# whh1747012859/Enhanced-UNet

Measured on AMD Instinct MI355X. Metric: training images/sec at 1024×1024 1-ch→2-cls, 1/2/4/8 MI355X; Dice vs CPU ref, higher is better.
Workload: dtype bf16

## Files before the change

### enhanced-unet_amd/csrc/bn_pool_up.hip

```cpp
#include "common.h"

#include <algorithm>

EUNET_DEBUG_UNIT(bnpool)

namespace {

constexpr int NT = 256;
constexpr int STH = 8, STW = 32;
constexpr int SFH = 16;
constexpr int SCI = 8;
constexpr int SJT = (SCI * 9 + 15) / 16;

struct SmallArgs {
  const void* x; int N, H, W, xct, xco, cin;
  const float* w; const float* b;
  void* y; int yct, yco, cout;
  float* stats; int tx, ty, ntiles;
};

template <typename T, bool C1>
__global__ __launch_bounds__(NT) void conv_small_fwd_kernel(SmallArgs a) {
  __shared__ float xs[(SFH + 2) * (STW + 2) * SCI];
  __shared__ __attribute__((aligned(16))) float wsm[SCI * 9 * 64];
// ... 341 lines not shown
  if (tid == 0 && c == 0 && nbt != nullptr) *nbt += 1;
  if (tid == 0) {
    const double var_b = m2 / n;
    const double var_u = n > 1.0 ? m2 / (n - 1.0) : var_b;
    const double istd = 1.0 / sqrt(var_b + (double)eps);
    const double sc = (double)gamma[c] * istd;
    if (mean_o) mean_o[c] = (float)mean;
    if (invstd_o) invstd_o[c] = (float)istd;
    if (scale_o) scale_o[c] = (float)sc;
    if (shift_o) shift_o[c] = (float)((double)beta[c] - mean * sc);
    if (rm) rm[c] = (float)((1.0 - mom) * (double)rm[c] + mom * mean);
    if (rv) rv[c] = (float)((1.0 - mom) * (double)rv[c] + mom * var_u);
  }
}

__global__ void bn_eval_affine_kernel(int C, const float* g, const float* b, const float* rm, const float* rv,
                                      float eps, float* sc, float* sh) {
  const int c = blockIdx.x * blockDim.x + threadIdx.x;
  if (c >= C) return;
  const float s = g[c] / sqrtf(rv[c] + eps);
  sc[c] = s;
  sh[c] = b[c] - rm[c] * s;
}

template <typename T>
__global__ void bnrelu_pool_kernel(const T* y, int N, int H, int W, int C, int yct, int yco, const float* sc,
                                   const float* sh, T* act, int act_ct, int act_co, T* pool, int pct, int pco) {
  constexpr int E = Vec16<T>::N;
  const int U = C / E, Ho = H / 2, Wo = W / 2;
  const long long id = (long long)blockIdx.x * blockDim.x + threadIdx.x;
// ... 306 lines not shown
  const int col = blockIdx.x * 64 + cl;
  double s = 0.0;
  if (col < cols) {
    for (int r = rg; r < rb; r += 32) {
      double v[8];
#pragma unroll
      for (int i = 0; i < 8; ++i) {
        const double x = ws[(long long)min(r + 4 * i, rb - 1) * cols + col];
        v[i] = r + 4 * i < rb ? x : 0.0;
      }
#pragma unroll
      for (int i = 0; i < 8; ++i) s += v[i];
    }
  }
  sh[rg][cl] = s;
  __syncthreads();
  if (rg == 0 && col < cols) {
    const float v = (float)(sh[0][cl] + sh[1][cl] + sh[2][cl] + sh[3][cl]);
    int i = 0;
#pragma unroll
    for (int j = 1; j < 4; ++j) i = (j < segs.n && col >= segs.start[j]) ? j : i;
    segs.out[i][col - segs.start[i]] = v;
  }
}

struct BnBwdCoef { float k1, kq, k2, k3; };
__device__ __forceinline__ BnBwdCoef bn_bwd_coef(float mean, float istd, float scale, float shift, float dbeta,
                                                 float dgamma, float inv_n) {
  const float off = -mean * istd;
  const float dg = dgamma * inv_n;
// ... 628 lines not shown
  for (int i = 0; i < segs.n; ++i)
    EUNET_REQUIRE(segs.out[i] && (i == 0 || (segs.start[i] > segs.start[i - 1] && segs.start[i] < cols)),
                  "colsum: bad segments");
  const int rb = colsum_rb(rows);
  const int chunk = cdiv(rows, rb);
  colsum_stage1<<<dim3(cdiv(cols, 64), rb), NT, 0, s>>>(part, rows, cols, ld, chunk, (double*)ws);
  colsum_stage2<<<cdiv(cols, 64), NT, 0, s>>>((const double*)ws, rb, cols, segs);
  EUNET_LAUNCH_CHECK("colsum");
  return EUNET_OK;
}

int eunet_colsum_ld(const float* part, int rows, int cols, int ld, float* out, void* ws, hipStream_t s, int split,
                    float* out_hi) {
  ColSegs g = {{out, out_hi, nullptr, nullptr}, {0, split, 0, 0}, out_hi != nullptr ? 2 : 1};
  return eunet_colsum_segs(part, rows, cols, ld, g, ws, s);
}

namespace {
int bnr_block(const eunet_act* g) {
  const int U = g->c / elems16(g->dtype);
  return U > 0 && NT % U == 0 ? NT : (U > 0 && 192 % U == 0 ? 192 : 0);
}
bool bnr_ok(const eunet_act* g, const eunet_act* y) {
  return act_ok(y) && vec_ok(y) && like(y, g) && bnr_block(g) > 0;
}
long long pool_threads(const eunet_act* gout) {
  return (long long)gout->n * (gout->h / 2) * (gout->w / 2) * (gout->c / elems16(gout->dtype));
}
int bnr_grid(long long threads, int cap, int block) { return (int)std::min<long long>((threads + block - 1) / block, cap); }
long long up_threads(const eunet_act* glo) {
// ... 212 lines not shown
  });
  EUNET_LAUNCH_CHECK("bn_bwd_reduce");
  return EUNET_OK;
}

int eunet_colsum_ws_bytes(int rows, int cols, size_t* bytes) {
  EUNET_REQUIRE(bytes && rows > 0 && cols > 0, "colsum_ws_bytes: bad args");
  *bytes = eunet_colsum_ws(rows, cols);
  return EUNET_OK;
}

int eunet_colsum(const float* part, int rows, int cols, float* out, void* ws, void* stream) {
  return eunet_colsum_ld(part, rows, cols, cols, out, ws, (hipStream_t)stream);
}

int eunet_colsum_split(const float* part, int rows, int cols, int split, float* out_lo, float* out_hi, void* ws,
                       void* stream) {
  EUNET_REQUIRE(out_hi && split > 0 && split < cols, "colsum_split: bad split");
  return eunet_colsum_ld(part, rows, cols, cols, out_lo, ws, (hipStream_t)stream, split, out_hi);
}

int eunet_bn_bwd_apply(const eunet_act* g, const eunet_act* y, const float* mean, const float* invstd,
                       const float* scale, const float* shift, const float* dbeta, const float* dgamma,
                       const eunet_act* gy, void* stream) {
  EUNET_REQUIRE(act_ok(g) && act_ok(y) && act_ok(gy) && vec_ok(g) && vec_ok(y) && vec_ok(gy),
                "bn_bwd_apply: bad tensors");
  EUNET_REQUIRE(mean && invstd && scale && shift && dbeta && dgamma, "bn_bwd_apply: null stats");
  EUNET_REQUIRE(like(g, y) && like(gy, y), "bn_bwd_apply: mismatch");
  const long long P = (long long)y->n * y->h * y->w;
  const int U = y->c / elems16(y->dtype);
// ... 171 lines not shown
```

### enhanced-unet_amd/csrc/common.h

```cpp
#pragma once
#include <hip/hip_runtime.h>

#include <mutex>
#include <utility>
#include <vector>
#include <stdint.h>
#include <stdio.h>
#include <string.h>

#include "../../include/eunet.h"

typedef __bf16 bf16x8 __attribute__((ext_vector_type(8)));
typedef short s16x4 __attribute__((ext_vector_type(4)));
typedef short s16x8 __attribute__((ext_vector_type(8)));
typedef float f32x4 __attribute__((ext_vector_type(4)));
typedef uint32_t u32x4 __attribute__((ext_vector_type(4)));
typedef float f32x2 __attribute__((ext_vector_type(2)));
typedef short s16x2 __attribute__((ext_vector_type(2)));
typedef uint16_t bf16_t;

__device__ __forceinline__ bf16x8 cat_bf16x4(s16x4 lo, s16x4 hi) {
  const s16x8 v = __builtin_shufflevector(lo, hi, 0, 1, 2, 3, 4, 5, 6, 7);
  return __builtin_bit_cast(bf16x8, v);
}
// ... 167 lines not shown
  f32x4 w = {0.25f, 0.75f, 0.75f, 0.25f};
  if (i == 0) { w[0] = 0.f; w[1] = 1.f; }
  if (i == in - 1) { w[2] = 1.f; w[3] = 0.f; }
  return w;
}

int eunet_colsum_ld(const float* part, int rows, int cols, int ld, float* out, void* ws, hipStream_t s,
                    int split = 0, float* out_hi = nullptr);
struct ColSegs {
  float* out[4];
  int start[4];
  int n;
};
int eunet_colsum_segs(const float* part, int rows, int cols, int ld, const ColSegs& segs, void* ws, hipStream_t s);

template <typename K>
inline void allow_lds(K* kernel, size_t bytes) {
  if (bytes <= 65536) return;
  static std::mutex mu;
  static std::vector<std::pair<const void*, size_t>> done;
  std::lock_guard<std::mutex> lock(mu);
  for (const auto& d : done)
    if (d.first == (const void*)kernel && d.second >= bytes) return;
  (void)hipFuncSetAttribute((const void*)kernel, hipFuncAttributeMaxDynamicSharedMemorySize, (int)bytes);
  done.emplace_back((const void*)kernel, bytes);
}

__host__ __device__ inline int cdiv(int a, int b) { return (a + b - 1) / b; }

inline bool act_ok(const eunet_act* a) {
// ... 27 lines not shown
```

### enhanced-unet_amd/eunet/_lib.py

```python
from __future__ import annotations

import ctypes
import os
from ctypes import POINTER, c_float, c_int, c_size_t, c_void_p, c_char_p, c_int64

LIB_PATH = os.environ.get("EUNET_LIB") or os.path.join(os.path.dirname(os.path.abspath(__file__)), "libeunet_hip.so")

EUNET_F32 = 0
EUNET_BF16 = 1


class Act(ctypes.Structure):
    _fields_ = [("ptr", c_void_p), ("n", c_int), ("h", c_int), ("w", c_int), ("c", c_int),
                ("ctot", c_int), ("coff", c_int), ("dtype", c_int)]


class PackDesc(ctypes.Structure):
    _fields_ = [("w", c_void_p), ("cout", c_int), ("cin", c_int), ("flip", c_int), ("wp", c_void_p)]


PACK_MAX = 32


class LossParams(ctypes.Structure):
# ... 82 lines not shown
    "eunet_bce_dice_bwd": [_f, _f, c_int, c_int, c_int, c_int, POINTER(BCEDiceParams), _f, _f, _f, c_void_p],
    "eunet_border_weight_map": [_f, _f, c_int, c_int, c_int, POINTER(c_float * 3), c_float, c_float, c_int, _f, c_void_p],
    "eunet_separate_instances": [_f, _f, c_int, c_int, c_int, _f, _f, c_void_p],
    "eunet_loss_fwd_w": [_f, _f, _f, c_int, c_int, c_int, c_int, POINTER(LossParams), _f, _f, _f, _f, c_void_p],
    "eunet_loss_bwd_w": [_f, _f, _f, c_int, c_int, c_int, c_int, POINTER(LossParams), _f, _f, _f, c_void_p],
    "eunet_bce_dice_fwd_w": [_f, _f, _f, c_int, c_int, c_int, c_int, POINTER(BCEDiceParams), _f, _f, _f, _f, c_void_p],
    "eunet_bce_dice_bwd_w": [_f, _f, _f, c_int, c_int, c_int, c_int, POINTER(BCEDiceParams), _f, _f, _f, c_void_p],
    "eunet_warp_grid": [_f, c_int, c_int, POINTER(ctypes.c_double * 6), c_int, c_int, _f, c_void_p],
    "eunet_warp_u8": [_f, c_int, c_int, c_int, _f, c_int, c_int, c_int, c_int, _f, c_void_p],
    "eunet_warp_labels": [_f, c_int, c_int, c_int, c_int, _f, c_int, c_int, c_int, c_int64, c_int, c_int, _f, c_void_p],
    "eunet_bn_bwd_tiles": [_P, POINTER(c_int)],
    "eunet_bn_bwd_reduce": [_P, _P, _f, _f, _f, _f, _f, c_void_p],
    "eunet_colsum_ws_bytes": [c_int, c_int, POINTER(c_size_t)],
    "eunet_colsum": [_f, c_int, c_int, _f, _f, c_void_p],
    "eunet_colsum_split": [_f, c_int, c_int, c_int, _f, _f, _f, c_void_p],
    "eunet_bn_bwd_apply": [_P, _P, _f, _f, _f, _f, _f, _f, _P, c_void_p],
    "eunet_bn_bwd_apply_1x1": [_P, _f, c_int, _f, _f, _f, _f, _f, _f, _f, _P, c_void_p],
    "eunet_pool_bwd_add": [_P, _P, _P, _P, c_void_p],
    "eunet_upsample_bwd": [_P, _P, c_void_p],
    "eunet_pool_bwd_add_bnr_rows": [_P, POINTER(c_int)],
    "eunet_pool_bwd_add_bnr": [_P, _P, _P, _P, _P, _f, _f, _f, _f, _f, c_void_p],
    "eunet_bn_bwd_apply_pool": [_P, _P, _P, _f, _f, _f, _f, _f, _f, _P, c_void_p],
    "eunet_upsample_bwd_bnr_rows": [_P, POINTER(c_int)],
    "eunet_upsample_bwd_bnr": [_P, _P, _P, _f, _f, _f, _f, _f, c_void_p],
    "eunet_conv1x1_bwd_tiles": [_P, POINTER(c_int)],
    "eunet_conv1x1_bwd": [_P, _f, _f, _f, c_int, _f, _P, _f, c_void_p],
    "eunet_conv1x1_bwd_bnr": [_P, _f, _f, _f, c_int, _f, _P, _f, _f, _f, _f, c_void_p],
    "eunet_semantic_counts": [_f, _f, c_int, c_int64, _f, c_void_p],
    "eunet_binary_overlap": [_f, _f, c_int64, _f, c_void_p],
    "eunet_resize_bilinear": [_f, c_int, c_int, c_int, _f, c_int, c_int, c_float, c_float, c_int, c_int,
# ... 166 lines not shown
```

### enhanced-unet_amd/eunet/dual.py

```python
from __future__ import annotations

from typing import List, Optional

import torch

from . import ops
from .engine import BN_EPS, BN_MOMENTUM, GradSink, UNetEngine, _e

DROP_P = (0.2, 0.15)
HEAD_CH = (256, 128, 64)
BRANCHES = ("unetpp", "deeplab")


class DualEngine:
    narrow_mfma = True

    def __init__(self, model):
        self.m = model
        self.K = model.num_classes
        self.ea = UNetEngine(model, prefix="unetpp.")
        self.eb = UNetEngine(model, prefix="deeplab.")
        self.drop_keep = None
        self.keep_state = False

# ... 73 lines not shown
        else:
            keep = torch.empty((N, C), dtype=torch.float32, device=dev).bernoulli_(1.0 - DROP_P[i])
        sc, sh, gs = (_e((N, C), torch.float32, dev) for _ in range(3))
        ops.dropout_affine(h["scale"], h["shift"], keep, DROP_P[i], sc, sh, gs)
        return dict(scale=sc, shift=sh, nstride=C, gscale=gs)

    def _bn_back(self, prefix, g, y, bn, P, sink, part=None, tiles=0):
        C = y.shape[3]
        dev = y.device
        if part is None:
            tiles = ops.bn_bwd_tiles(ops.act(y))
            part = _e(tiles * 2 * C, torch.float32, dev)
            ops.bn_bwd_reduce(ops.act(g), ops.act(y), bn["mean"], bn["invstd"], bn["scale"],
                              bn["shift"], part)
        dbeta, dgamma = sink.slot(prefix + ".bias", (C,)), sink.slot(prefix + ".weight", (C,))
        ops.colsum(part, tiles, 2 * C, dbeta, split=C, out_hi=dgamma)
        gy = torch.empty_like(y)
        ops.bn_bwd_apply(ops.act(g), ops.act(y), bn["mean"], bn["invstd"], bn["scale"],
                         bn["shift"], dbeta, dgamma, ops.act(gy))
        return gy

    def _wgrad(self, name, xa: ops.Act, gy, sink, d=None):
        C = gy.shape[3]
        dev = gy.device
        gya = ops.act(gy)
        ns = ops.conv3x3_wgrad_splits(gya, xa.c, self.dtype)
        dwp = _e(ns * C * 9 * xa.c, torch.float32, dev)
        ops.conv3x3_wgrad(xa, gya, dwp, None, ns, scale=d["scale"], shift=d["shift"], nstride=d["nstride"])
        ops.wgrad_reduce(dwp, None, ns, C, xa.c, 9, sink.slot(name, (C, xa.c, 3, 3)), None)

    def backward(self, S, g_out, g_aux_a, g_aux_b, sink: Optional[GradSink] = None):
# ... 2 lines not shown
        N, H, W = S["N"], S["H"], S["W"]
        dev = g_out.device
        sink = sink or GradSink(dev)
        za, zb = S["SA"]["z"], S["SB"]["z"]
        tiles, gtiles = ops.fusion_tiles(N, H, W)
        g1, g2, h1, h2, h3, d1, d2 = (S[k] for k in ("g1", "g2", "h1", "h2", "h3", "d1", "d2"))
        y1, y2, y3, a, b, f2 = (S[k] for k in ("y1", "y2", "y3", "a", "b", "f2"))
        g_out = g_out.contiguous().float()
        gz = _e((N, H, W, K), torch.float32, dev)
        gf2res = _e((N, H, W, 2 * K), torch.float32, dev)
        nv = K * 2 * K + K
        part = _e(tiles * nv, torch.float32, dev)
        ops.fusion_out_bwd(za, zb, K, g_out, b, g2["scale"], g2["shift"],
                           P["fusion_residual.weight"].reshape(K, 2 * K).contiguous(), gz, gf2res, part)
        red = _e(nv, torch.float32, dev)
        ops.colsum(part, tiles, nv, red)
        sink.slot("fusion_residual.weight", (K, 2 * K, 1, 1)).copy_(red[:2 * K * K].view(K, 2 * K, 1, 1))
        sink.slot("fusion_residual.bias", (K,)).copy_(red[2 * K * K:])
        C3 = HEAD_CH[2]
        g3 = torch.empty_like(y3)
        ct = ops.conv1x1_bwd_tiles(ops.act(y3))
        part = _e(ct * (K * C3 + K), torch.float32, dev)
        w11 = P["fusion_head.11.weight"].reshape(K, C3).contiguous()
        bpart = _e(ct * 2 * C3, torch.float32, dev)
        ops.conv1x1_bwd_bnr(ops.act(y3), h3["scale"], h3["shift"], w11, K, gz, ops.act(g3), part,
                            h3["mean"], h3["invstd"], bpart)
        red = _e(K * C3 + K, torch.float32, dev)
        ops.colsum(part, ct, K * C3 + K, red)
        sink.slot("fusion_head.11.weight", (K, C3, 1, 1)).copy_(red[:K * C3].view(K, C3, 1, 1))
        sink.slot("fusion_head.11.bias", (K,)).copy_(red[K * C3:])
        sink.ready(["fusion_residual.weight", "fusion_residual.bias", "fusion_head.11.weight", "fusion_head.11.bias"])
        gy3 = self._bn_back("fusion_head.9", g3, y3, h3, P, sink, part=bpart, tiles=ct)
        del g3
        self._wgrad("fusion_head.8.weight", ops.act(y2), gy3, sink, d2)
        gg2 = torch.empty_like(y2)
        ct = ops.conv3x3_tiles(ops.act(gg2))
        cpart = _e(ct * 2 * HEAD_CH[1], torch.float32, dev)
        ops.conv3x3_dgrad_bnbwd(ops.act(gy3), ops.conv3x3_pack(P["fusion_head.8.weight"], dt, flip=True),
                                ops.act(gg2), ops.act(y2), h2["mean"], h2["invstd"], h2["scale"],
                                h2["shift"], cpart, gscale=d2["gscale"])
        del gy3
        sink.ready(["fusion_head.9.weight", "fusion_head.9.bias", "fusion_head.8.weight"])
        gy2 = self._bn_back("fusion_head.5", gg2, y2, h2, P, sink, part=cpart, tiles=ct)
# ... 13 lines not shown
        ns = ops.conv_small_wgrad_splits(ops.act(gy1))
        dwp = _e(ns * HEAD_CH[0] * 9 * 2 * K, torch.float32, dev)
        ops.conv_small_wgrad(f2a, ops.act(gy1), dwp, None, ns)
        ops.wgrad_reduce(dwp, None, ns, HEAD_CH[0], 2 * K, 9, sink.slot("fusion_head.0.weight", (HEAD_CH[0], 2 * K, 3, 3)),
                         None)
        gf2c = _e((N, H, W, 8), torch.float32, dev)
        ops.conv3x3_dgrad(ops.act(gy1), ops.conv3x3_pack(P["fusion_head.0.weight"], dt, flip=True), ops.act(gf2c))
        del gy1
        sink.ready(["fusion_head.1.weight", "fusion_head.1.bias", "fusion_head.0.weight"])
        gffd = _e((N, H, W, 2 * K), torch.float32, dev)
        gbhat = _e((N, H, W, 2 * K), torch.float32, dev)
        part = _e(tiles * 4 * K, torch.float32, dev)
        ops.gate_bwd1(za, zb, K, ops.act(gf2c), gf2res, b, g2["mean"], g2["invstd"], P["attention_gate.4.weight"],
                      P["attention_gate.4.bias"], gffd, gbhat, part)
        red2 = _e(4 * K, torch.float32, dev)
        ops.colsum(part, tiles, 4 * K, red2)
        sink.slot("attention_gate.4.bias", (2 * K,)).copy_(red2[:2 * K])
        sink.slot("attention_gate.4.weight", (2 * K,)).copy_(red2[2 * K:])
        nv = 2 * K * K + 2 * K
        gabn = _e((N, H, W, K), torch.float32, dev)
        part = _e(tiles * nv, torch.float32, dev)
        ops.gate_bwd2(N, H, W, K, gbhat, b, g2["mean"], g2["invstd"], P["attention_gate.4.weight"], red2[:2 * K],
                      red2[2 * K:], a, g1["mean"], g1["invstd"], P["attention_gate.1.weight"],
                      P["attention_gate.1.bias"], P["attention_gate.3.weight"].reshape(2 * K, K).contiguous(), gabn,
                      part)
        red1 = _e(nv, torch.float32, dev)
        ops.colsum(part, tiles, nv, red1)
        sink.slot("attention_gate.3.weight", (2 * K, K, 1, 1)).copy_(red1[:2 * K * K].view(2 * K, K, 1, 1))
        db1, dg1 = red1[2 * K * K:2 * K * K + K], red1[2 * K * K + K:]
        sink.slot("attention_gate.1.bias", (K,)).copy_(db1)
        sink.slot("attention_gate.1.weight", (K,)).copy_(dg1)
        gz_a = _e((N, H, W, K), torch.float32, dev)
        gz_b = _e((N, H, W, K), torch.float32, dev)
        nw = K * 2 * K * 9
        part = _e(gtiles * nw, torch.float32, dev)
        ops.gate_bwd3(za, zb, K, gabn, a, g1["mean"], g1["invstd"], P["attention_gate.1.weight"], db1, dg1,
                      P["attention_gate.0.weight"].contiguous(), gffd,
                      None if g_aux_a is None else g_aux_a.contiguous().float(),
                      None if g_aux_b is None else g_aux_b.contiguous().float(), gz_a, gz_b, part)
        ops.colsum(part, gtiles, nw, sink.slot("attention_gate.0.weight", (K, 2 * K, 3, 3)).view(-1))
        sink.ready(["attention_gate.4.weight", "attention_gate.4.bias", "attention_gate.3.weight",
                    "attention_gate.1.weight", "attention_gate.1.bias", "attention_gate.0.weight"])
        self.ea.backward_trunk(S["SA"], gz_a, sink)
        self.eb.backward_trunk(S["SB"], gz_b, sink)
        return sink.finish()


def dual_backward_order(model) -> List[str]:
    names = [n for n, _ in model.named_parameters()]
    head = ["fusion_residual.weight", "fusion_residual.bias", "fusion_head.11.weight", "fusion_head.11.bias",
            "fusion_head.9.weight", "fusion_head.9.bias", "fusion_head.8.weight",
            "fusion_head.5.weight", "fusion_head.5.bias", "fusion_head.4.weight",
            "fusion_head.1.weight", "fusion_head.1.bias", "fusion_head.0.weight",
            "attention_gate.4.weight", "attention_gate.4.bias", "attention_gate.3.weight",
            "attention_gate.1.weight", "attention_gate.1.bias", "attention_gate.0.weight"]
# ... 33 lines not shown
```

### enhanced-unet_amd/eunet/engine.py

```python
from __future__ import annotations

from typing import Dict, Optional

import torch

from . import kprof, ops
from ._lib import EunetError

ENCODER_SCOPE = "conv3x3.encoder_train"

BLOCKS = ("enc1", "enc2", "enc3", "enc4", "dec4", "dec3", "dec2")
UPCONVS = ("up4", "up3", "up2")
BN_EPS = 1e-5
BN_MOMENTUM = 0.1
class Grad1x1:

    def __init__(self, w, k, gz):
        self.w, self.k, self.gz = w, k, gz


class GradPool:

    def __init__(self, gpool, gskip):
        self.gpool, self.gskip = gpool, gskip
# ... 27 lines not shown
def side_stream(device) -> torch.cuda.Stream:
    key = torch.device(device).index
    if key not in _SIDE:
        _SIDE[key] = torch.cuda.Stream(device=device)
    return _SIDE[key]


class UNetEngine:

    overlap_wgrad = True
    materialize_za = False
    dec1_recompute = True
    pool_recompute = True
    device_fence_forks = True
    keep_state = False

    def _wait(self, to, frm):
        if self.device_fence_forks:
            ops.stream_wait(frm, to)
        else:
            to.wait_stream(frm)

    def __init__(self, model, prefix: str = "model."):
        self.m = model
        self.prefix = prefix
        self.base = model.base_ch
        self.K = model.num_classes
        self.cin = model.in_channels
        self.dtype = model.compute_dtype
        self.transpose = getattr(model, "upsample", "bilinear") == "transpose"

    def _P(self):
        return dict(self.m.named_parameters())

    def _B(self):
        return dict(self.m.named_buffers())

    def _bn(self, prefix, stats, tiles, C, training, P, B):
        dev = P[prefix + ".weight"].device
        scale, shift = _e(C, torch.float32, dev), _e(C, torch.float32, dev)
        if training:
            mean, invstd = _e(C, torch.float32, dev), _e(C, torch.float32, dev)
            ops.bn_finalize(stats, tiles, C, P[prefix + ".weight"], P[prefix + ".bias"], BN_EPS, BN_MOMENTUM,
                            B[prefix + ".running_mean"], B[prefix + ".running_var"], mean, invstd, scale, shift,
                            B[prefix + ".num_batches_tracked"])
            return dict(mean=mean, invstd=invstd, scale=scale, shift=shift)
        ops.bn_eval_affine(P[prefix + ".weight"], P[prefix + ".bias"], B[prefix + ".running_mean"],
                           B[prefix + ".running_var"], BN_EPS, scale, shift)
        return dict(mean=None, invstd=None, scale=scale, shift=shift)

    def _stats_buf(self, y):
        tiles = ops.conv3x3_tiles(ops.act(y))
        C = y.shape[3]
        return _e(tiles * (2 * C + 1), torch.float32, y.device), tiles

    def _pack_all(self, P, training: bool):
        items, names = [], []
        for nm in BLOCKS:
            p = f"{self.prefix}{nm}"
            for i in ((3,) if nm == "enc1" else (0, 3)):
# ... 123 lines not shown
    def _block_bwd(self, nm, G, S, P, sink, need_gx: bool, small: bool, gred=(None, 0)):
        with kprof.scope(ENCODER_SCOPE if nm.startswith("enc") else None):
            return self._block_bwd_impl(nm, G, S, P, sink, need_gx, small, gred)

    def _block_bwd_impl(self, nm, G: "torch.Tensor | Grad1x1 | GradPool", S, P, sink: GradSink, need_gx: bool,
                        small: bool, gred=(None, 0)):
        p = f"{self.prefix}{nm}"
        s = S[nm]
        ya, yb, bna, bnb, X = s["ya"], s["yb"], s["bna"], s["bnb"], s["X"]
        N, H, W, C = yb.shape
        dev, dt = yb.device, self.dtype

        def bn_back(prefix, g, y, bn, part=None, tiles=0):
            if isinstance(g, (Grad1x1, GradPool)):
                dbeta, dgamma = sink.slot(prefix + ".bias", (C,)), sink.slot(prefix + ".weight", (C,))
                ops.colsum(part, tiles, 2 * C, dbeta, split=C, out_hi=dgamma)
                gy = torch.empty_like(y)
                if isinstance(g, Grad1x1):
                    ops.bn_bwd_apply_1x1(ops.act(y), g.w, g.k, g.gz, bn["mean"], bn["invstd"], bn["scale"],
                                         bn["shift"], dbeta, dgamma, ops.act(gy))
                else:
                    ops.bn_bwd_apply_pool(g.gpool, g.gskip, ops.act(y), bn["mean"], bn["invstd"], bn["scale"],
                                          bn["shift"], dbeta, dgamma, ops.act(gy))
                return gy
            if part is None:
                tiles = ops.bn_bwd_tiles(ops.act(y))
                part = _e(tiles * 2 * C, torch.float32, dev)
                ops.bn_bwd_reduce(ops.act(g), ops.act(y), bn["mean"], bn["invstd"], bn["scale"],
                                  bn["shift"], part)
            dbeta, dgamma = sink.slot(prefix + ".bias", (C,)), sink.slot(prefix + ".weight", (C,))
            ops.colsum(part, tiles, 2 * C, dbeta, split=C, out_hi=dgamma)
            gy = torch.empty_like(y)
            ops.bn_bwd_apply(ops.act(g), ops.act(y), bn["mean"], bn["invstd"], bn["scale"],
                             bn["shift"], dbeta, dgamma, ops.act(gy))
            return gy

        main = torch.cuda.current_stream(dev)
        side = side_stream(dev) if self.overlap_wgrad else None

        def wgrad(conv, xa: ops.Act, gy, scale=None, shift=None, small_conv=False, on_main=False):
            dw = sink.slot(conv + ".weight", (C, xa.c, 3, 3))
            db = sink.slot(conv + ".bias", (C,))
            if side is None or on_main:
                return wgrad_on_stream(xa, gy, dw, db, scale, shift, small_conv)
            self._wait(side, main)
            with torch.cuda.stream(side):
# ... 87 lines not shown

        def upconv_bwd(ghi: ops.Act, glo: torch.Tensor, nm, up):
            s = S[nm]
            C = glo.shape[3]
            ops.upconv2x2_dgrad(ghi, S["up"][up], ops.act(glo))
            names = [f"{pre}{up}.weight", f"{pre}{up}.bias"]
            dw, db = sink.slot(names[0], (C, C, 2, 2)), sink.slot(names[1], (C,))

            def wgrad():
                ya = ops.act(s["yb"])
                ns = ops.upconv2x2_wgrad_splits(ya, dt)
                dwp = _e(ns * 4 * C * C, torch.float32, dev)
                dbp = _e(ns * 4 * C, torch.float32, dev)
                ops.upconv2x2_wgrad(ya, s["bnb"]["scale"], s["bnb"]["shift"], ghi, dwp, dbp, ns)
                ops.wgrad_reduce(dwp, None, ns, C, C, 4, dw, None)
                ops.colsum(dbp, ns * 4, C, db)
                sink.ready(names)

            if not self.overlap_wgrad:
                wgrad()
                return None, 0
            main, side = torch.cuda.current_stream(dev), side_stream(dev)
            self._wait(side, main)
            with torch.cuda.stream(side):
                wgrad()
            for t in (ghi._keep, s["yb"], dw, db):
                t.record_stream(side)
            return None, 0

        def up_bwd(ghi: ops.Act, glo: torch.Tensor, nm, up):
            if self.transpose:
# ... 24 lines not shown
        yb_act = ops.act(s2["yb"])
        tiles = ops.conv1x1_bwd_tiles(yb_act)
        part = _e(tiles * (K * b + K), torch.float32, dev)
        w1 = P[pre + "dec1.weight"].reshape(K, b).contiguous()
        bnb2 = s2["bnb"]
        bpart = _e(tiles * 2 * b, torch.float32, dev)
        if self.dec1_recompute:
            gd2 = Grad1x1(w1, K, gz)
            ops.conv1x1_bwd_bnr(yb_act, bnb2["scale"], bnb2["shift"], w1, K, gz, None, part,
                                bnb2["mean"], bnb2["invstd"], bpart)
        else:
            gd2 = torch.empty_like(s2["yb"])
            ops.conv1x1_bwd_bnr(yb_act, bnb2["scale"], bnb2["shift"], w1, K, gz, ops.act(gd2), part,
                                bnb2["mean"], bnb2["invstd"], bpart)
        red2 = (bpart, tiles)
        ops.colsum(part, tiles, K * b + K, sink.slot(pre + "dec1.weight", (K, b, 1, 1)), split=K * b,
                   out_hi=sink.slot(pre + "dec1.bias", (K,)))
        sink.ready([pre + "dec1.weight", pre + "dec1.bias"])
        g_cat2 = self._block_bwd("dec2", gd2, S, P, sink, need_gx=True, small=False, gred=red2)
        del gd2
        g_d3 = _e((N, H >> 1, W >> 1, ch[1]), dt, dev)
        red = up_bwd(ops.act(g_cat2, 0, ch[1]), g_d3, "dec3", "up2")
        g_cat3 = self._block_bwd("dec3", g_d3, S, P, sink, need_gx=True, small=False, gred=red)
        del g_d3
        g_d4 = _e((N, H >> 2, W >> 2, ch[2]), dt, dev)
        red = up_bwd(ops.act(g_cat3, 0, ch[2]), g_d4, "dec4", "up3")
        g_cat4 = self._block_bwd("dec4", g_d4, S, P, sink, need_gx=True, small=False, gred=red)
        del g_d4
        g_e4 = _e((N, H >> 3, W >> 3, ch[3]), dt, dev)
        red = up_bwd(ops.act(g_cat4, 0, ch[3]), g_e4, "enc4", "up4")
        g_p3 = self._block_bwd("enc4", g_e4, S, P, sink, need_gx=True, small=False, gred=red)
        del g_e4
# ... 38 lines not shown
```

### enhanced-unet_amd/eunet/ops.py

```python
from __future__ import annotations

import ctypes
import math

import torch

from . import _lib, kprof
from ._lib import Act, call, c_int, c_size_t

DTYPES = {torch.float32: _lib.EUNET_F32, torch.bfloat16: _lib.EUNET_BF16}

USE_DISPATCHER = True
_LIB = torch.library.Library("eunet", "DEF")
DISPATCHED: dict = {}


def _dispatched(kinds: str, returns_tensor: bool = False):
    import inspect
    import string

    ks = kinds.split()

    def deco(fn):
        sig = inspect.signature(fn)
# ... 221 lines not shown
             _ptr(stats), _stream())


def conv_small_wgrad_splits(dy: Act) -> int:
    s = c_int()
    call("eunet_conv_small_wgrad_splits", ctypes.byref(dy), ctypes.byref(s))
    return s.value


@_dispatched("A A T! T!? i")
def conv_small_wgrad(x: Act, dy: Act, dw_part, db_part, nsplit):
    call("eunet_conv_small_wgrad", ctypes.byref(x), ctypes.byref(dy), _ptr(dw_part), _ptr(db_part), nsplit,
         _stream())


@_dispatched("T i i T T f f T!? T!? T!? T!? T!? T!? T!?")
def bn_finalize(stats, tiles, c, gamma, beta, eps, momentum, run_mean, run_var, mean, invstd, scale, shift,
                num_batches_tracked=None):
    call("eunet_bn_finalize", _ptr(stats), tiles, c, _ptr(gamma), _ptr(beta), float(eps), float(momentum),
         _ptr(run_mean), _ptr(run_var), _ptr(mean), _ptr(invstd), _ptr(scale), _ptr(shift),
         _ptr(num_batches_tracked), _stream())


@_dispatched("T T T T f T! T!")
def bn_eval_affine(gamma, beta, run_mean, run_var, eps, scale, shift):
    call("eunet_bn_eval_affine", gamma.numel(), _ptr(gamma), _ptr(beta), _ptr(run_mean), _ptr(run_var),
         float(eps), _ptr(scale), _ptr(shift), _stream())


@_dispatched("A T T A!")
def bnrelu(y: Act, scale, shift, out: Act):
    call("eunet_bnrelu", ctypes.byref(y), _ptr(scale), _ptr(shift), ctypes.byref(out), _stream())

# ... 272 lines not shown
    return lo, so


def bn_bwd_tiles(y: Act) -> int:
    t = c_int()
    call("eunet_bn_bwd_tiles", ctypes.byref(y), ctypes.byref(t))
    return t.value


@_dispatched("A A T T T T T!")
def bn_bwd_reduce(g: Act, y: Act, mean, invstd, scale, shift, part):
    call("eunet_bn_bwd_reduce", ctypes.byref(g), ctypes.byref(y), _ptr(mean), _ptr(invstd), _ptr(scale),
         _ptr(shift), _ptr(part), _stream())


@_dispatched("T i i T! i? T!?")
def colsum(part, rows, cols, out, split=None, out_hi=None):
    b = c_size_t()
    call("eunet_colsum_ws_bytes", rows, cols, ctypes.byref(b))
    ws = torch.empty(b.value, dtype=torch.uint8, device=part.device)
    if out_hi is None:
        call("eunet_colsum", _ptr(part), rows, cols, _ptr(out), _ptr(ws), _stream())
    else:
        call("eunet_colsum_split", _ptr(part), rows, cols, int(split), _ptr(out), _ptr(out_hi), _ptr(ws), _stream())


@_dispatched("A A T T T T T T A!")
def bn_bwd_apply(g: Act, y: Act, mean, invstd, scale, shift, dbeta, dgamma, gy: Act):
    call("eunet_bn_bwd_apply", ctypes.byref(g), ctypes.byref(y), _ptr(mean), _ptr(invstd), _ptr(scale),
         _ptr(shift), _ptr(dbeta), _ptr(dgamma), ctypes.byref(gy), _stream())


# ... 1395 lines not shown
```

### include/eunet.h

```cpp
#ifndef EUNET_H
#define EUNET_H

#include <stddef.h>
#include <stdint.h>

#ifdef __cplusplus
extern "C" {
#endif

#define EUNET_OK 0
#define EUNET_ERR_INVALID (-1)
#define EUNET_ERR_HIP (-2)

enum { EUNET_F32 = 0, EUNET_BF16 = 1 };

typedef struct {
  void* ptr;
  int n, h, w;
  int c;
  int ctot;
  int coff;
  int dtype;
} eunet_act;

// ... 31 lines not shown
                        int in_nstride, const eunet_act* dy, float* dw_part, float* db_part, int nsplit,
                        void* stream);
int eunet_wgrad_reduce(const float* dw_part, const float* db_part, int nsplit, int cout, int cin,
                       int taps, float* dw, float* db, void* stream);

int eunet_conv_small_fwd(const eunet_act* x, const float* w, const float* bias,
                         const eunet_act* y, float* stats, void* stream);
int eunet_conv_small_wgrad_splits(const eunet_act* dy, int* nsplit);
int eunet_conv_small_wgrad(const eunet_act* x, const eunet_act* dy, float* dw_part,
                           float* db_part, int nsplit, void* stream);

int eunet_bn_finalize(const float* stats, int tiles, int c, const float* gamma, const float* beta,
                      float eps, float momentum, float* run_mean, float* run_var, float* mean,
                      float* invstd, float* scale, float* shift, int64_t* num_batches_tracked,
                      void* stream);
int eunet_bn_eval_affine(int c, const float* gamma, const float* beta, const float* run_mean,
                         const float* run_var, float eps, float* scale, float* shift, void* stream);

int eunet_bnrelu(const eunet_act* y, const float* scale, const float* shift, const eunet_act* out, void* stream);

int eunet_bnrelu_pool(const eunet_act* y, const float* scale, const float* shift,
                      const eunet_act* act, const eunet_act* pooled, void* stream);
int eunet_bnrelu_upsample(const eunet_act* y, const float* scale, const float* shift,
                          const eunet_act* out, void* stream);
int eunet_upconv2x2_packed_bytes(int c, int dtype, size_t* bytes);
int eunet_upconv2x2_pack(const float* w, int c, void* wp, int dtype, void* stream);
int eunet_bnrelu_upconv2x2_fwd(const eunet_act* y, const float* scale, const float* shift, const void* wp,
                               const float* bias, const eunet_act* out, void* stream);
int eunet_upconv2x2_dgrad(const eunet_act* g, const void* wp, const eunet_act* gd, void* stream);
int eunet_upconv2x2_wgrad_splits(const eunet_act* y, int dtype, int* nsplit);
// ... 84 lines not shown
#define EUNET_WARP_CONSTANT 0
#define EUNET_WARP_REFLECT101 1
int eunet_warp_u8(const uint8_t* src, int hi, int wi, int c, const float* grid, int ho, int wo, int border,
                  int fill, uint8_t* dst, void* stream);
int eunet_warp_labels(const void* src, int elem_bytes, int planes, int hi, int wi, const float* grid, int ho,
                      int wo, int border, long long fill, int flip_h, int flip_v, void* dst, void* stream);

int eunet_bn_bwd_tiles(const eunet_act* y, int* tiles);
int eunet_bn_bwd_reduce(const eunet_act* g, const eunet_act* y, const float* mean,
                        const float* invstd, const float* scale, const float* shift, float* part,
                        void* stream);
int eunet_colsum_ws_bytes(int rows, int cols, size_t* bytes);
int eunet_colsum(const float* part, int rows, int cols, float* out, void* ws, void* stream);
int eunet_colsum_split(const float* part, int rows, int cols, int split, float* out_lo,
                       float* out_hi, void* ws, void* stream);
int eunet_bn_bwd_apply(const eunet_act* g, const eunet_act* y, const float* mean,
                       const float* invstd, const float* scale, const float* shift,
                       const float* dbeta, const float* dgamma, const eunet_act* gy,
                       void* stream);
int eunet_debug_enabled(void);
int eunet_debug_status(unsigned* unit_line, unsigned* count, int reset);
int eunet_debug_selftest(void* stream);
int eunet_pool_bwd_add(const eunet_act* act, const eunet_act* gpool, const eunet_act* gskip,
                       const eunet_act* gout, void* stream);
int eunet_upsample_bwd(const eunet_act* ghi, const eunet_act* glo, void* stream);
int eunet_pool_bwd_add_bnr_rows(const eunet_act* gout, int* rows);
int eunet_pool_bwd_add_bnr(const eunet_act* act, const eunet_act* gpool, const eunet_act* gskip,
                           const eunet_act* gout, const eunet_act* y, const float* mean, const float* invstd,
                           const float* scale, const float* shift, float* part, void* stream);
int eunet_bn_bwd_apply_pool(const eunet_act* gpool, const eunet_act* gskip, const eunet_act* y, const float* mean,
// ... 218 lines not shown
```

Baseline: 194.4.

## Fuse two-stage colsum and BN finalize into single launches with last-block tickets

Replaces the two-kernel column-sum reduction with one kernel: each block publishes its partial to a workspace, and the last block to finish (found via an atomic ticket counter) does the final reduction. It also adds a multi-block BN finalize that spreads large tile counts across 64 blocks per channel group and merges Welford stats in the last block. Workspaces are cached per device and stream to avoid allocating each call. This saves a kernel launch and a round of serialization per reduction, at the cost of atomics, fences, and a persistent counter state that must reset correctly.

```diff
diff --git a/enhanced-unet_amd/csrc/bn_pool_up.hip b/enhanced-unet_amd/csrc/bn_pool_up.hip
--- a/enhanced-unet_amd/csrc/bn_pool_up.hip
+++ b/enhanced-unet_amd/csrc/bn_pool_up.hip
@@ -379,6 +379,98 @@
   }
 }
 
+constexpr int FCLS = 64;
+__global__ __launch_bounds__(FNT) void bn_finalize_classes_kernel(const float* st, int tiles, int C,
+                                                                 const float* gamma, const float* beta, float eps,
+                                                                 float mom, float* rm, float* rv, float* mean_o,
+                                                                 float* invstd_o, float* scale_o, float* shift_o,
+                                                                 long long* nbt, const double* guard, double* rec,
+                                                                 unsigned* cnt) {
+  __shared__ double shn[FNT], shm[FNT], shq[FNT];
+  __shared__ int last;
+  const int tid = threadIdx.x, cl = tid & 63, k = tid >> 6;
+  const int j = blockIdx.x, grp = blockIdx.y;
+  const int c = min(grp * 64 + cl, C - 1);
+  const float* cnt_t = st + (long long)2 * C * tiles;
+  double n = 0.0, mean = 0.0, m2 = 0.0;
+  auto merge = [](double& n, double& mean, double& m2, double nb, double mb, double qb) {
+    const double nt = n + nb;
+    if (nb <= 0.0) return;
+    const double d = mb - mean;
+    mean += d * (nb / nt);
+    m2 += qb + d * d * (n * nb / nt);
+    n = nt;
+  };
+  constexpr int FB = 8;
+  for (int t0 = j + FCLS * k; t0 < tiles; t0 += FB * FNT) {
+    float vn[FB], vs[FB], vq[FB];
+#pragma unroll
+    for (int i = 0; i < FB; ++i) {
+      const bool in = t0 + i * FNT < tiles;
+      const long long ti = min(t0 + i * FNT, tiles - 1);
+      const float a = cnt_t[ti], b = st[(ti * 2) * C + c], q = st[(ti * 2 + 1) * C + c];
+      vn[i] = in ? a : 0.f;
+      vs[i] = in ? b : 0.f;
+      vq[i] = in ? q : 0.f;
+    }
+#pragma unroll
+    for (int i = 0; i < FB; ++i) {
+      const double nb = (double)vn[i];
+      if (nb > 0.0) merge(n, mean, m2, nb, (double)vs[i] / nb, (double)vq[i]);
+    }
+  }
+  shn[tid] = n; shm[tid] = mean; shq[tid] = m2;
+  __syncthreads();
+  for (int o = FNT / 2; o >= FCLS; o >>= 1) {
+    if (tid < o) {
+      double a_n = shn[tid], a_m = shm[tid], a_q = shq[tid];
+      merge(a_n, a_m, a_q, shn[tid + o], shm[tid + o], shq[tid + o]);
+      shn[tid] = a_n; shm[tid] = a_m; shq[tid] = a_q;
+    }
+    __syncthreads();
+  }
+  double* rg = rec + (long long)grp * 3 * 64 * FCLS;
+  if (k == 0) {
+    publish(rg + (0 * 64 + cl) * FCLS + j, shn[cl]);
+    publish(rg + (1 * 64 + cl) * FCLS + j, shm[cl]);
+    publish(rg + (2 * 64 + cl) * FCLS + j, shq[cl]);
+  }
+  if (!ticket_last(&cnt[grp], FCLS, &last)) return;
+  const bool keep = guard != nullptr && *guard != 0.0;
+  if (keep) { rm = nullptr; rv = nullptr; nbt = nullptr; }
+  if (tid == 0 && grp == 0 && nbt != nullptr) *nbt += 1;
+  const int cc = tid >> 4, q = tid & 15;
+  double rn[4], rmn[4], rq[4];
+#pragma unroll
+  for (int i = 0; i < 4; ++i) {
+    rn[i] = rg[(0 * 64 + cc) * FCLS + q + 16 * i];
+    rmn[i] = rg[(1 * 64 + cc) * FCLS + q + 16 * i];
+    rq[i] = rg[(2 * 64 + cc) * FCLS + q + 16 * i];
+  }
+  merge(rn[0], rmn[0], rq[0], rn[2], rmn[2], rq[2]);
+  merge(rn[1], rmn[1], rq[1], rn[3], rmn[3], rq[3]);
+  merge(rn[0], rmn[0], rq[0], rn[1], rmn[1], rq[1]);
+  n = rn[0]; mean = rmn[0]; m2 = rq[0];
+#pragma unroll
+  for (int o = 8; o > 0; o >>= 1) {
+    const double bn = __shfl_down(n, o, 16), bm = __shfl_down(mean, o, 16), bq = __shfl_down(m2, o, 16);
+    merge(n, mean, m2, bn, bm, bq);
+  }
+  const int ch = grp * 64 + cc;
+  if (q == 0 && ch < C) {
+    const double var_b = m2 / n;
+    const double var_u = n > 1.0 ? m2 / (n - 1.0) : var_b;
+    const double istd = 1.0 / sqrt(var_b + (double)eps);
+    const double sc = (double)gamma[ch] * istd;
+    if (mean_o) mean_o[ch] = (float)mean;
+    if (invstd_o) invstd_o[ch] = (float)istd;
+    if (scale_o) scale_o[ch] = (float)sc;
+    if (shift_o) shift_o[ch] = (float)((double)beta[ch] - mean * sc);
+    if (rm) rm[ch] = (float)((1.0 - mom) * (double)rm[ch] + mom * mean);
+    if (rv) rv[ch] = (float)((1.0 - mom) * (double)rv[ch] + mom * var_u);
+  }
+}
+
 __global__ void bn_eval_affine_kernel(int C, const float* g, const float* b, const float* rm, const float* rv,
                                       float eps, float* sc, float* sh) {
   const int c = blockIdx.x * blockDim.x + threadIdx.x;
@@ -715,6 +807,45 @@
     }
   }
   sh[rg][cl] = s;
+  __syncthreads();
+  if (rg == 0 && col < cols) {
+    const float v = (float)(sh[0][cl] + sh[1][cl] + sh[2][cl] + sh[3][cl]);
+    int i = 0;
+#pragma unroll
+    for (int j = 1; j < 4; ++j) i = (j < segs.n && col >= segs.start[j]) ? j : i;
+    segs.out[i][col - segs.start[i]] = v;
+  }
+}
+
+template <typename T>
+__device__ __forceinline__ double colsum_group(const T* src, int first, int r1, long long ld, int col) {
+  double s = 0.0;
+  for (int r = first; r < r1; r += 32) {
+    T v[8];
+#pragma unroll
+    for (int i = 0; i < 8; ++i) {
+      const T x = src[(long long)min(r + 4 * i, r1 - 1) * ld + col];
+      v[i] = r + 4 * i < r1 ? x : (T)0;
+    }
+#pragma unroll
+    for (int i = 0; i < 8; ++i) s += (double)v[i];
+  }
+  return s;
+}
+
+__global__ __launch_bounds__(NT) void colsum_fused_kernel(const float* part, int rows, int cols, int ld, int chunk,
+                                                          double* ws, unsigned* cnt, ColSegs segs) {
+  __shared__ double sh[4][64];
+  __shared__ int last;
+  const int tid = threadIdx.x, cl = tid & 63, rg = tid >> 6;
+  const int col = blockIdx.x * 64 + cl;
+  const int r0 = blockIdx.y * chunk, r1 = min(rows, r0 + chunk);
+  sh[rg][cl] = col < cols ? colsum_group(part, r0 + rg, r1, ld, col) : 0.0;
+  __syncthreads();
+  if (rg == 0 && col < cols)
+    publish(&ws[(long long)blockIdx.y * cols + col], sh[0][cl] + sh[1][cl] + sh[2][cl] + sh[3][cl]);
+  if (!ticket_last(&cnt[blockIdx.x], gridDim.y, &last)) return;
+  sh[rg][cl] = col < cols ? colsum_group((const double*)ws, rg, (int)gridDim.y, cols, col) : 0.0;
   __syncthreads();
   if (rg == 0 && col < cols) {
     const float v = (float)(sh[0][cl] + sh[1][cl] + sh[2][cl] + sh[3][cl]);
@@ -1373,6 +1504,20 @@
                     float* out_hi) {
   ColSegs g = {{out, out_hi, nullptr, nullptr}, {0, split, 0, 0}, out_hi != nullptr ? 2 : 1};
   return eunet_colsum_segs(part, rows, cols, ld, g, ws, s);
+}
+
+static int colsum_fused(const float* part, int rows, int cols, int split, float* out, float* out_hi, void* ws,
+                        hipStream_t s) {
+  EUNET_REQUIRE(part && out && ws && rows > 0 && cols > 0 && cdiv(cols, 64) <= TICKET_WORDS, "colsum_fused: bad args");
+  EUNET_REQUIRE(out_hi == nullptr || (split > 0 && split < cols), "colsum_fused: bad split");
+  const ColSegs g = {{out, out_hi, nullptr, nullptr}, {0, split, 0, 0}, out_hi != nullptr ? 2 : 1};
+  const int rb = colsum_rb(rows);
+  const int chunk = cdiv(rows, rb);
+  unsigned* cnt = (unsigned*)ws;
+  colsum_fused_kernel<<<dim3(cdiv(cols, 64), rb), NT, 0, s>>>(part, rows, cols, cols, chunk,
+                                                             (double*)(cnt + TICKET_WORDS), cnt, g);
+  EUNET_LAUNCH_CHECK("colsum_fused");
+  return EUNET_OK;
 }
 
 namespace {
@@ -1615,6 +1760,36 @@
   return eunet_colsum_ld(part, rows, cols, cols, out, ws, (hipStream_t)stream);
 }
 
+int eunet_colsum_fused_ws_bytes(int rows, int cols, size_t* bytes) {
+  EUNET_REQUIRE(bytes && rows > 0 && cols > 0, "colsum_fused_ws_bytes: bad args");
+  *bytes = TICKET_WORDS * sizeof(unsigned) + eunet_colsum_ws(rows, cols);
+  return EUNET_OK;
+}
+
+int eunet_colsum_fused(const float* part, int rows, int cols, int split, float* out_lo, float* out_hi, void* ws,
+                       void* stream) {
+  return colsum_fused(part, rows, cols, split, out_lo, out_hi, ws, (hipStream_t)stream);
+}
+
+int eunet_bn_finalize_classes_ws_bytes(int c, size_t* bytes) {
+  EUNET_REQUIRE(bytes && c > 0, "bn_finalize_classes_ws_bytes: bad args");
+  *bytes = TICKET_WORDS * sizeof(unsigned) + (size_t)cdiv(c, 64) * FCLS * 3 * 64 * sizeof(double);
+  return EUNET_OK;
+}
+
+int eunet_bn_finalize_classes(const float* stats, int tiles, int c, const float* gamma, const float* beta, float eps,
+                              float momentum, float* run_mean, float* run_var, float* mean, float* invstd,
+                              float* scale, float* shift, int64_t* num_batches_tracked, void* ws, void* stream) {
+  EUNET_REQUIRE(stats && tiles > 0 && c > 0 && gamma && beta && ws && cdiv(c, 64) <= TICKET_WORDS,
+                "bn_finalize_classes: bad args");
+  unsigned* cnt = (unsigned*)ws;
+  bn_finalize_classes_kernel<<<dim3(FCLS, cdiv(c, 64)), FNT, 0, (hipStream_t)stream>>>(
+      stats, tiles, c, gamma, beta, eps, momentum, run_mean, run_var, mean, invstd, scale, shift,
+      (long long*)num_batches_tracked, eunet::update_guard(), (double*)(cnt + TICKET_WORDS), cnt);
+  EUNET_LAUNCH_CHECK("bn_finalize_classes");
+  return EUNET_OK;
+}
+
 int eunet_colsum_split(const float* part, int rows, int cols, int split, float* out_lo, float* out_hi, void* ws,
                        void* stream) {
   EUNET_REQUIRE(out_hi && split > 0 && split < cols, "colsum_split: bad split");
diff --git a/enhanced-unet_amd/csrc/common.h b/enhanced-unet_amd/csrc/common.h
--- a/enhanced-unet_amd/csrc/common.h
+++ b/enhanced-unet_amd/csrc/common.h
@@ -205,6 +205,27 @@
 };
 int eunet_colsum_segs(const float* part, int rows, int cols, int ld, const ColSegs& segs, void* ws, hipStream_t s);
 
+constexpr int TICKET_WORDS = 512;
+template <typename T>
+__device__ __forceinline__ void publish(T* p, T v) {
+  __hip_atomic_store(p, v, __ATOMIC_RELAXED, __HIP_MEMORY_SCOPE_AGENT);
+}
+__device__ __forceinline__ bool ticket_last(unsigned* cnt, unsigned n, int* flag ) {
+  asm volatile("s_waitcnt vmcnt(0)" ::: "memory");
+  __syncthreads();
+  if (threadIdx.x == 0) {
+    const bool last = __hip_atomic_fetch_add(cnt, 1u, __ATOMIC_RELAXED, __HIP_MEMORY_SCOPE_AGENT) == n - 1;
+    if (last) {
+      __hip_atomic_store(cnt, 0u, __ATOMIC_RELAXED, __HIP_MEMORY_SCOPE_AGENT);
+      __builtin_amdgcn_fence(__ATOMIC_ACQUIRE, "agent");
+      asm volatile("s_waitcnt vmcnt(0)" ::: "memory");
+    }
+    *flag = last;
+  }
+  __syncthreads();
+  return *flag != 0;
+}
+
 template <typename K>
 inline void allow_lds(K* kernel, size_t bytes) {
   if (bytes <= 65536) return;
diff --git a/enhanced-unet_amd/eunet/_lib.py b/enhanced-unet_amd/eunet/_lib.py
--- a/enhanced-unet_amd/eunet/_lib.py
+++ b/enhanced-unet_amd/eunet/_lib.py
@@ -120,6 +120,11 @@
     "eunet_colsum_ws_bytes": [c_int, c_int, POINTER(c_size_t)],
     "eunet_colsum": [_f, c_int, c_int, _f, _f, c_void_p],
     "eunet_colsum_split": [_f, c_int, c_int, c_int, _f, _f, _f, c_void_p],
+    "eunet_colsum_fused_ws_bytes": [c_int, c_int, POINTER(c_size_t)],
+    "eunet_colsum_fused": [_f, c_int, c_int, c_int, _f, _f, _f, c_void_p],
+    "eunet_bn_finalize_classes_ws_bytes": [c_int, POINTER(c_size_t)],
+    "eunet_bn_finalize_classes": [_f, c_int, c_int, _f, _f, c_float, c_float, _f, _f, _f, _f, _f, _f, _f, _f,
+                                  c_void_p],
     "eunet_bn_bwd_apply": [_P, _P, _f, _f, _f, _f, _f, _f, _P, c_void_p],
     "eunet_bn_bwd_apply_1x1": [_P, _f, c_int, _f, _f, _f, _f, _f, _f, _f, _P, c_void_p],
     "eunet_pool_bwd_add": [_P, _P, _P, _P, c_void_p],
diff --git a/enhanced-unet_amd/eunet/dual.py b/enhanced-unet_amd/eunet/dual.py
--- a/enhanced-unet_amd/eunet/dual.py
+++ b/enhanced-unet_amd/eunet/dual.py
@@ -111,7 +111,7 @@
             ops.bn_bwd_reduce(ops.act(g), ops.act(y), bn["mean"], bn["invstd"], bn["scale"],
                               bn["shift"], part)
         dbeta, dgamma = sink.slot(prefix + ".bias", (C,)), sink.slot(prefix + ".weight", (C,))
-        ops.colsum(part, tiles, 2 * C, dbeta, split=C, out_hi=dgamma)
+        self.ea._colsum(part, tiles, 2 * C, dbeta, split=C, out_hi=dgamma)
         gy = torch.empty_like(y)
         ops.bn_bwd_apply(ops.act(g), ops.act(y), bn["mean"], bn["invstd"], bn["scale"],
                          bn["shift"], dbeta, dgamma, ops.act(gy))
@@ -144,7 +144,7 @@
         ops.fusion_out_bwd(za, zb, K, g_out, b, g2["scale"], g2["shift"],
                            P["fusion_residual.weight"].reshape(K, 2 * K).contiguous(), gz, gf2res, part)
         red = _e(nv, torch.float32, dev)
-        ops.colsum(part, tiles, nv, red)
+        self.ea._colsum(part, tiles, nv, red)
         sink.slot("fusion_residual.weight", (K, 2 * K, 1, 1)).copy_(red[:2 * K * K].view(K, 2 * K, 1, 1))
         sink.slot("fusion_residual.bias", (K,)).copy_(red[2 * K * K:])
         C3 = HEAD_CH[2]
@@ -156,7 +156,7 @@
         ops.conv1x1_bwd_bnr(ops.act(y3), h3["scale"], h3["shift"], w11, K, gz, ops.act(g3), part,
                             h3["mean"], h3["invstd"], bpart)
         red = _e(K * C3 + K, torch.float32, dev)
-        ops.colsum(part, ct, K * C3 + K, red)
+        self.ea._colsum(part, ct, K * C3 + K, red)
         sink.slot("fusion_head.11.weight", (K, C3, 1, 1)).copy_(red[:K * C3].view(K, C3, 1, 1))
         sink.slot("fusion_head.11.bias", (K,)).copy_(red[K * C3:])
         sink.ready(["fusion_residual.weight", "fusion_residual.bias", "fusion_head.11.weight", "fusion_head.11.bias"])
@@ -200,7 +200,7 @@
         ops.gate_bwd1(za, zb, K, ops.act(gf2c), gf2res, b, g2["mean"], g2["invstd"], P["attention_gate.4.weight"],
                       P["attention_gate.4.bias"], gffd, gbhat, part)
         red2 = _e(4 * K, torch.float32, dev)
-        ops.colsum(part, tiles, 4 * K, red2)
+        self.ea._colsum(part, tiles, 4 * K, red2)
         sink.slot("attention_gate.4.bias", (2 * K,)).copy_(red2[:2 * K])
         sink.slot("attention_gate.4.weight", (2 * K,)).copy_(red2[2 * K:])
         nv = 2 * K * K + 2 * K
@@ -211,7 +211,7 @@
                       P["attention_gate.1.bias"], P["attention_gate.3.weight"].reshape(2 * K, K).contiguous(), gabn,
                       part)
         red1 = _e(nv, torch.float32, dev)
-        ops.colsum(part, tiles, nv, red1)
+        self.ea._colsum(part, tiles, nv, red1)
         sink.slot("attention_gate.3.weight", (2 * K, K, 1, 1)).copy_(red1[:2 * K * K].view(2 * K, K, 1, 1))
         db1, dg1 = red1[2 * K * K:2 * K * K + K], red1[2 * K * K + K:]
         sink.slot("attention_gate.1.bias", (K,)).copy_(db1)
@@ -224,7 +224,7 @@
                       P["attention_gate.0.weight"].contiguous(), gffd,
                       None if g_aux_a is None else g_aux_a.contiguous().float(),
                       None if g_aux_b is None else g_aux_b.contiguous().float(), gz_a, gz_b, part)
-        ops.colsum(part, gtiles, nw, sink.slot("attention_gate.0.weight", (K, 2 * K, 3, 3)).view(-1))
+        self.ea._colsum(part, gtiles, nw, sink.slot("attention_gate.0.weight", (K, 2 * K, 3, 3)).view(-1))
         sink.ready(["attention_gate.4.weight", "attention_gate.4.bias", "attention_gate.3.weight",
                     "attention_gate.1.weight", "attention_gate.1.bias", "attention_gate.0.weight"])
         self.ea.backward_trunk(S["SA"], gz_a, sink)
diff --git a/enhanced-unet_amd/eunet/engine.py b/enhanced-unet_amd/eunet/engine.py
--- a/enhanced-unet_amd/eunet/engine.py
+++ b/enhanced-unet_amd/eunet/engine.py
@@ -65,6 +65,12 @@
     pool_recompute = True
     device_fence_forks = True
     keep_state = False
+    one_launch_reduce = True
+    FINALIZE_CLASSES_TILES = 4096
+
+    def _colsum(self, part, rows, cols, out, split=None, out_hi=None):
+        ws = ops.ticket_ws(part.device, ops.colsum_ws_bytes(rows, cols)) if self.one_launch_reduce else None
+        ops.colsum(part, rows, cols, out, split=split, out_hi=out_hi, ws=ws)
 
     def _wait(self, to, frm):
         if self.device_fence_forks:
@@ -94,7 +100,9 @@
             mean, invstd = _e(C, torch.float32, dev), _e(C, torch.float32, dev)
             ops.bn_finalize(stats, tiles, C, P[prefix + ".weight"], P[prefix + ".bias"], BN_EPS, BN_MOMENTUM,
                             B[prefix + ".running_mean"], B[prefix + ".running_var"], mean, invstd, scale, shift,
-                            B[prefix + ".num_batches_tracked"])
+                            B[prefix + ".num_batches_tracked"],
+                            ws=ops.ticket_ws(dev, ops.bn_finalize_ws_bytes(C))
+                            if self.one_launch_reduce and tiles >= self.FINALIZE_CLASSES_TILES else None)
             return dict(mean=mean, invstd=invstd, scale=scale, shift=shift)
         ops.bn_eval_affine(P[prefix + ".weight"], P[prefix + ".bias"], B[prefix + ".running_mean"],
                            B[prefix + ".running_var"], BN_EPS, scale, shift)
@@ -248,7 +256,7 @@
         def bn_back(prefix, g, y, bn, part=None, tiles=0):
             if isinstance(g, (Grad1x1, GradPool)):
                 dbeta, dgamma = sink.slot(prefix + ".bias", (C,)), sink.slot(prefix + ".weight", (C,))
-                ops.colsum(part, tiles, 2 * C, dbeta, split=C, out_hi=dgamma)
+                self._colsum(part, tiles, 2 * C, dbeta, split=C, out_hi=dgamma)
                 gy = torch.empty_like(y)
                 if isinstance(g, Grad1x1):
                     ops.bn_bwd_apply_1x1(ops.act(y), g.w, g.k, g.gz, bn["mean"], bn["invstd"], bn["scale"],
@@ -263,7 +271,7 @@
                 ops.bn_bwd_reduce(ops.act(g), ops.act(y), bn["mean"], bn["invstd"], bn["scale"],
                                   bn["shift"], part)
             dbeta, dgamma = sink.slot(prefix + ".bias", (C,)), sink.slot(prefix + ".weight", (C,))
-            ops.colsum(part, tiles, 2 * C, dbeta, split=C, out_hi=dgamma)
+            self._colsum(part, tiles, 2 * C, dbeta, split=C, out_hi=dgamma)
             gy = torch.empty_like(y)
             ops.bn_bwd_apply(ops.act(g), ops.act(y), bn["mean"], bn["invstd"], bn["scale"],
                              bn["shift"], dbeta, dgamma, ops.act(gy))
@@ -381,7 +389,7 @@
                 dbp = _e(ns * 4 * C, torch.float32, dev)
                 ops.upconv2x2_wgrad(ya, s["bnb"]["scale"], s["bnb"]["shift"], ghi, dwp, dbp, ns)
                 ops.wgrad_reduce(dwp, None, ns, C, C, 4, dw, None)
-                ops.colsum(dbp, ns * 4, C, db)
+                self._colsum(dbp, ns * 4, C, db)
                 sink.ready(names)
 
             if not self.overlap_wgrad:
@@ -436,8 +444,8 @@
             ops.conv1x1_bwd_bnr(yb_act, bnb2["scale"], bnb2["shift"], w1, K, gz, ops.act(gd2), part,
                                 bnb2["mean"], bnb2["invstd"], bpart)
         red2 = (bpart, tiles)
-        ops.colsum(part, tiles, K * b + K, sink.slot(pre + "dec1.weight", (K, b, 1, 1)), split=K * b,
-                   out_hi=sink.slot(pre + "dec1.bias", (K,)))
+        self._colsum(part, tiles, K * b + K, sink.slot(pre + "dec1.weight", (K, b, 1, 1)), split=K * b,
+                     out_hi=sink.slot(pre + "dec1.bias", (K,)))
         sink.ready([pre + "dec1.weight", pre + "dec1.bias"])
         g_cat2 = self._block_bwd("dec2", gd2, S, P, sink, need_gx=True, small=False, gred=red2)
         del gd2
diff --git a/enhanced-unet_amd/eunet/ops.py b/enhanced-unet_amd/eunet/ops.py
--- a/enhanced-unet_amd/eunet/ops.py
+++ b/enhanced-unet_amd/eunet/ops.py
@@ -1,6 +1,7 @@
 from __future__ import annotations
 
 import ctypes
+import functools
 import math
 
 import torch
@@ -259,9 +260,43 @@
          _stream())
 
 
-@_dispatched("T i i T T f f T!? T!? T!? T!? T!? T!? T!?")
+_TICKET_WS = {}
+
+
+def ticket_ws(device, nbytes: int) -> torch.Tensor:
+    dev = torch.device(device)
+    idx = dev.index if dev.index is not None else torch.cuda.current_device()
+    key = (idx, torch.cuda.current_stream(dev).cuda_stream)
+    ws = _TICKET_WS.get(key)
+    if ws is None or ws.numel() < nbytes:
+        ws = _TICKET_WS[key] = torch.zeros(max(int(nbytes), 1 << 20), dtype=torch.uint8, device=dev)
+    return ws
+
+
+@functools.lru_cache(maxsize=None)
+def bn_finalize_ws_bytes(c: int) -> int:
+    b = c_size_t()
+    call("eunet_bn_finalize_classes_ws_bytes", int(c), ctypes.byref(b))
+    return b.value
+
+
+@functools.lru_cache(maxsize=None)
+def colsum_ws_bytes(rows: int, cols: int) -> int:
+    b = c_size_t()
+    call("eunet_colsum_fused_ws_bytes", int(rows), int(cols), ctypes.byref(b))
+    return b.value
+
+
+@_dispatched("T i i T T f f T!? T!? T!? T!? T!? T!? T!? T!?")
 def bn_finalize(stats, tiles, c, gamma, beta, eps, momentum, run_mean, run_var, mean, invstd, scale, shift,
-                num_batches_tracked=None):
+                num_batches_tracked=None, ws=None):
+    if ws is not None:
+        if ws.numel() * ws.element_size() < bn_finalize_ws_bytes(c):
+            raise _lib.EunetError(f"bn_finalize: ws needs {bn_finalize_ws_bytes(c)} bytes")
+        call("eunet_bn_finalize_classes", _ptr(stats), tiles, c, _ptr(gamma), _ptr(beta), float(eps),
+             float(momentum), _ptr(run_mean), _ptr(run_var), _ptr(mean), _ptr(invstd), _ptr(scale), _ptr(shift),
+             _ptr(num_batches_tracked), _ptr(ws), _stream())
+        return
     call("eunet_bn_finalize", _ptr(stats), tiles, c, _ptr(gamma), _ptr(beta), float(eps), float(momentum),
          _ptr(run_mean), _ptr(run_var), _ptr(mean), _ptr(invstd), _ptr(scale), _ptr(shift),
          _ptr(num_batches_tracked), _stream())
@@ -564,8 +599,14 @@
          _ptr(shift), _ptr(part), _stream())
 
 
-@_dispatched("T i i T! i? T!?")
-def colsum(part, rows, cols, out, split=None, out_hi=None):
+@_dispatched("T i i T! i? T!? T!?")
+def colsum(part, rows, cols, out, split=None, out_hi=None, ws=None):
+    if ws is not None:
+        if ws.numel() * ws.element_size() < colsum_ws_bytes(rows, cols):
+            raise _lib.EunetError(f"colsum: ws needs {colsum_ws_bytes(rows, cols)} bytes")
+        call("eunet_colsum_fused", _ptr(part), rows, cols, 0 if out_hi is None else int(split), _ptr(out),
+             _ptr(out_hi), _ptr(ws), _stream())
+        return
     b = c_size_t()
     call("eunet_colsum_ws_bytes", rows, cols, ctypes.byref(b))
     ws = torch.empty(b.value, dtype=torch.uint8, device=part.device)
diff --git a/include/eunet.h b/include/eunet.h
--- a/include/eunet.h
+++ b/include/eunet.h
@@ -69,6 +69,11 @@
                       float eps, float momentum, float* run_mean, float* run_var, float* mean,
                       float* invstd, float* scale, float* shift, int64_t* num_batches_tracked,
                       void* stream);
+int eunet_bn_finalize_classes_ws_bytes(int c, size_t* bytes);
+int eunet_bn_finalize_classes(const float* stats, int tiles, int c, const float* gamma, const float* beta,
+                              float eps, float momentum, float* run_mean, float* run_var, float* mean,
+                              float* invstd, float* scale, float* shift, int64_t* num_batches_tracked,
+                              void* ws, void* stream);
 int eunet_bn_eval_affine(int c, const float* gamma, const float* beta, const float* run_mean,
                          const float* run_var, float eps, float* scale, float* shift, void* stream);
 
@@ -183,6 +188,9 @@
 int eunet_colsum(const float* part, int rows, int cols, float* out, void* ws, void* stream);
 int eunet_colsum_split(const float* part, int rows, int cols, int split, float* out_lo,
                        float* out_hi, void* ws, void* stream);
+int eunet_colsum_fused_ws_bytes(int rows, int cols, size_t* bytes);
+int eunet_colsum_fused(const float* part, int rows, int cols, int split, float* out_lo, float* out_hi,
+                       void* ws, void* stream);
 int eunet_bn_bwd_apply(const eunet_act* g, const eunet_act* y, const float* mean,
                        const float* invstd, const float* scale, const float* shift,
                        const float* dbeta, const float* dgamma, const eunet_act* gy,
```

Result: slower. 191.7 (-1.4%).
